# C-bowman/inference-tools

Measured on AMD Instinct MI355X. Metric: GpRegressor fit+predict wall-time and GFLOP/s at N=16384, d=8; % fp64 MFMA peak, higher is better.
Workload: dtype f64

## Files before the change

inference-tools_amd/csrc/api.hip:

```cpp
#include "api_internal.h"
#include <malloc.h>


thread_local std::string g_create_err;


int lane_streams(gpmi_ctx* c, Lane& L) {
  const size_t index = c->lanes.size() - 1;
  L.owns_stream = index < 2;
  if (!L.owns_stream) L.stream = c->lanes[index % 2].stream;
  if (L.owns_stream) HIPCHK(c, hipStreamCreateWithFlags(&L.stream, hipStreamNonBlocking));
  hipDeviceProp_t prop;
  HIPCHK(c, hipGetDeviceProperties(&prop, c->device));
  c->ncu = prop.multiProcessorCount;
  HIPCHK(c, hipEventCreateWithFlags(&L.ev_la, hipEventDisableTiming));
  HIPCHK(c, hipEventCreateWithFlags(&L.ev_panel, hipEventDisableTiming));
  HIPCHK(c, hipEventCreateWithFlags(&L.ev_join, hipEventDisableTiming));
  HIPCHK(c, hipEventCreateWithFlags(&L.ev_main, hipEventDisableTiming));
  HIPCHK(c, hipEventCreateWithFlags(&L.ev_slice, hipEventDisableTiming));
  return GPMI_OK;
}


bool ensure_masked_pair(gpmi_ctx* c, Lane& L, int k) {
// ... 240 lines not shown
      HIPCHK(c, hipStreamWaitEvent(su, L.ev_join, 0));
      launch_kbuild_square_part(s, p, c->x, c->n, c->np, c->noise, L.A, c->ld, 1, GPMI_OB);
      launch_kbuild_square_part(su, p, c->x, c->n, c->np, c->noise, L.A, c->ld, 2, GPMI_OB);
    } else {
      ProfScope ps(c, s, GPMI_PROF_KBUILD, 0.0, 4.0 * c->np * c->np);
      launch_kbuild_square(s, p, c->x, c->n, c->np, c->noise, L.A, c->ld, true);
    }
  }
  if (c->ycov) launch_add_full(s, L.A, c->ld, c->ycov, c->n);
  static const bool early_fill = !std::getenv("GPMI_EARLY_FILL") || std::atoi(std::getenv("GPMI_EARLY_FILL")) != 0;
  L.early = Lane::EarlyWork();
  L.early.pending = true;
  L.early.y = c->y;
  L.early.mu = mu_dev;
  L.early.mu_const = mu_const;
  L.early.r = L.vec + 2 * c->np;
  L.early.n = c->n;
  L.early.np = c->np;
  L.early.fill[0] = L.vec;
  L.early.fill[1] = backward_out;
  L.early.ident = early_identity;
  L.early.ident_ld = c->ld;
  L.identity_ready = false;
  if (!early_fill) L.early.pending = false;
  potrf_lower(c, L, L.A, c->np, c->ld, L.invD, L.info + slot, allow_lookahead);
  if (!early_fill) L.early.pending = true;
  lane_run_early(L, s);
  if (prebuild_inv2 && L.su[0] && c->np >= 4 * GPMI_OB) {
    HIPCHK(c, hipEventRecord(L.ev_join, s));
    HIPCHK(c, hipStreamWaitEvent(L.su[0], L.ev_join, 0));
    if (int rc = ensure_inv2(c, L, L.su[0])) return rc;
    HIPCHK(c, hipEventRecord(L.ev_main, L.su[0]));
  }
  trsv_forward(c, s, L.A, c->np, c->ld, L.invD, L.vec + 2 * c->np, L.vec, L.info + slot, BatchShape(), true);
  if (prebuild_inv2 && L.inv2_valid && L.su[0]) {
    HIPCHK(c, hipEventRecord(L.ev_la, s));
    HIPCHK(c, hipStreamWaitEvent(L.su[0], L.ev_la, 0));
    launch_lml_reduce(L.su[0], L.vec, L.A, c->ld, c->np, L.red + 2 * slot);
    HIPCHK(c, hipEventRecord(L.ev_main, L.su[0]));
  } else {
    launch_lml_reduce(s, L.vec, L.A, c->ld, c->np, L.red + 2 * slot);
  }
  HIPCHK(c, hipGetLastError());
  return GPMI_OK;
}

int ensure_second_matrix(gpmi_ctx* c, Lane& L) {
  if (!L.B2) HIPCHK(c, hipMalloc(&L.B2, sizeof(double) * c->np * c->ld));
  return GPMI_OK;
}

int ensure_inv2(gpmi_ctx* c, Lane& F, hipStream_t s) {
  if (F.inv2_valid) return GPMI_OK;
  const int64_t nob = (c->np / GPMI_NB + 3) / 4;
  if (!F.inv2) HIPCHK(c, hipMalloc(&F.inv2, sizeof(double) * nob * GPMI_OB * GPMI_OB));
  if (!F.inv2_t) HIPCHK(c, hipMalloc(&F.inv2_t, sizeof(double) * nob * 256 * 256));
  build_inv2(s, F.A, c->np, c->ld, F.invD, F.inv2, F.inv2_t);
// ... 598 lines not shown
```

inference-tools_amd/csrc/gemm_f64.hip:

```cpp
#include <cstdlib>

#include "gemm_tiles.h"

namespace {

using namespace gemm_tiles;

struct GemmArgs {
  double* C;
  const double* A;
  const double* B;
  int64_t ldc, lda, ldb;
  int ntr, ntc, k;
  int kskip;
  unsigned long long* stamp;
  int64_t sC, sA, sB;
  int split, tile_base;
  FlowHook hook;
  int zlocal_tiles;
  int mixed_full;
};

struct WgId {
  int wid;
  int64_t bz;
};
__device__ inline int xcd_remap(int b, int nwg);
__device__ inline WgId wg_id(int kskip, int zlocal_tiles) {
  if (zlocal_tiles > 0) {
    const int n = (int)blockIdx.x, m = n >> 3;
    return {m % zlocal_tiles, (int64_t)(m / zlocal_tiles) * 8 + (n & 7)};
  }
  return {kskip ? (int)blockIdx.x : xcd_remap(blockIdx.x, gridDim.x), (int64_t)blockIdx.z};
}


__device__ inline int xcd_remap(int b, int nwg) {
  const int q = nwg >> 3, r = nwg & 7, xcd = b & 7;
  return (xcd < r ? xcd * (q + 1) : r * (q + 1) + (xcd - r) * q) + (b >> 3);
}

template <int TILES>
__device__ inline void tile_of(int id, int ntr, int ntc, int& ti, int& tj) {
// ... 46 lines not shown
    tile_of<TILES>(g.tile_base + wid, g.ntr, g.ntc, ti, tj);
    if (TILES == TILES_RECT && (g.kskip == 2 || g.kskip == 4) && 2 * ti >= g.ntr) tj = g.ntc - 1 - tj;
  }

  const int tid = threadIdx.x;
  const bool stamp_first = g.stamp && tid == 0 && blockIdx.x < 8 && blockIdx.z == 0;
  if (stamp_first) g.stamp[blockIdx.x] = __builtin_amdgcn_s_memrealtime();
  const unsigned mid = gridDim.x >> 1;
  const bool stamp_clock = g.stamp && tid == 0 && blockIdx.x >= mid && blockIdx.x < mid + 8 && blockIdx.z == 0;
  unsigned long long c_start = 0, r_start = 0;
  if (stamp_clock) {
    r_start = __builtin_amdgcn_s_memrealtime();
    c_start = __builtin_amdgcn_s_memtime();
  }
  const int kbeg = (g.kskip == 1) ? ti * BM : (g.kskip == 4) ? tj * BN : 0;
  const int kend = (g.kskip == 2 && (tj + 1) * BN < g.k) ? (tj + 1) * BN : g.k;
  const int64_t bz = me.bz;
  const double* __restrict__ Ag = g.A + bz * g.sA + (int64_t)ti * BM * g.lda + kbeg;
  const double* __restrict__ Bg = BKN ? g.B + bz * g.sB + (int64_t)kbeg * g.ldb + (int64_t)tj * BN
                                      : g.B + bz * g.sB + (int64_t)tj * BN * g.ldb + kbeg;
  double* Cg = g.C + bz * g.sC + (int64_t)ti * BM * g.ldc + (int64_t)tj * BN;
  if constexpr (OP == OP_ASSIGN && BKN == 0 && BN == 128 && BM <= 64) {
    if (g.kskip == 3) {
      staged_tile<OP, BKN, BM, BN, CST_NT, LD_PLAIN, true>(Ag, Bg, Cg, g.lda, g.ldb, g.ldc, (kend - kbeg) / BK, smem);
    } else {
      staged_tile<OP, BKN, BM, BN>(Ag, Bg, Cg, g.lda, g.ldb, g.ldc, (kend - kbeg) / BK, smem);
    }
  } else {
    staged_tile<OP, BKN, BM, BN>(Ag, Bg, Cg, g.lda, g.ldb, g.ldc, (kend - kbeg) / BK, smem);
  }

  const bool stamp_end = g.stamp && tid == 0 && blockIdx.x + 1024 >= gridDim.x;
  if (stamp_end) {
    asm volatile("s_waitcnt vmcnt(0)" ::: "memory");
    g.stamp[8 + (__builtin_amdgcn_s_getreg(((4 - 1) << 11) | 20) & 7)] = __builtin_amdgcn_s_memrealtime();
  }
  if (stamp_clock)
    g.stamp[16 + blockIdx.x - mid] = ((__builtin_amdgcn_s_memtime() - c_start) << 32) |
                                     ((__builtin_amdgcn_s_memrealtime() - r_start) & 0xffffffffull);
}


#ifndef GPMI_DMA_WGS
#define GPMI_DMA_WGS 2
#endif
typedef __attribute__((address_space(3))) double gemm_lds_double_t;
typedef __attribute__((address_space(1))) double gemm_glb_double_t;
// ... 149 lines not shown
    } else if (!b_kmajor || op == OP_SUB) {
      bm = 64;
      bn = 64;
      if (tiles == TILES_RECT && !b_kmajor && k > 128 && big * 4 * bt.count <= m32_max && !bt.ring_order_only) bm = 32;
      static const bool bn32 = [] {
        const char* e = std::getenv("GPMI_CHAIN_BN32");
        return !e || std::atoi(e) != 0;
      }();
      if (bn32 && bm == 32 && kskip == 2 && op == OP_ASSIGN && big * 8 * bt.count <= 2 * 256) bn = 32;
    }
  }
  if (part == 0 && kskip == 4 && b_kmajor && op == OP_ASSIGN && tiles == TILES_RECT) {
    if (big * 16 * bt.count <= 2 * 256) {
      bm = 32;
      bn = 32;
    } else {
      bm = 64;
      bn = 128;
    }
  }
  if (bt.b_lower_tri && kskip == 0 && bn == 128 && bm <= 64 && ntc == 1 && k == 128 && !b_kmajor && op == OP_ASSIGN) kskip = 3;
  GemmArgs g{C, A, B, ldc, lda, ldb, ntr * (128 / bm), ntc * (128 / bn), k, kskip, stamp,
             bt.sC, bt.sA, bt.sB, part == 2 ? 1 : 0, (part == 2 || part == 3) ? (int)nfull : 0, bt.hook, 0, 0};
  int64_t nwg;
  if (tiles == TILES_RECT)
    nwg = (int64_t)g.ntr * g.ntc;
  else
    nwg = (int64_t)g.ntc * (g.ntc + 1) / 2 + (int64_t)(g.ntr - g.ntc) * g.ntc;
  if (part == 1) nwg = nfull;
  if (nend < 0 || nend > big) nend = big;
  if (part == 2) nwg = 4 * (nend - nfull);
  if (part == 3) nwg = nend - nfull;
  if (part == 4) {
    g.mixed_full = (int)nfull;
    nwg = nfull + 4 * (nend - nfull);
  }
  if (nwg <= 0) return;
  dim3 grid((unsigned)nwg, 1, (unsigned)bt.count), block(256);
  static const bool batch_xcd = [] {
    const char* e = std::getenv("GPMI_BATCH_XCD");
    return !e || std::atoi(e) != 0;
  }();
  if (batch_xcd && bt.count >= 8 && bt.count % 8 == 0 && !stamp && nwg * bt.count < (int64_t)1 << 30) {
    g.zlocal_tiles = (int)nwg;
    grid = dim3((unsigned)(nwg * bt.count), 1, 1);
  }
// ... 139 lines not shown
```

inference-tools_amd/csrc/gemm_tiles.h:

```cpp
#pragma once
#include "gpmi_internal.h"

#ifndef GPMI_C_PLAIN
#define GPMI_C_LOAD(p) __builtin_nontemporal_load(p)
#define GPMI_C_STORE(v, p) __builtin_nontemporal_store(v, p)
#else
#define GPMI_C_LOAD(p) (*(p))
#define GPMI_C_STORE(v, p) (*(p) = (v))
#endif

namespace gemm_tiles {

constexpr int CST_NT = 0, CST_SC1 = 1;
template <int CST>
__device__ __forceinline__ void c_store_begin() {
  if (CST == CST_SC1) asm volatile("s_nop 15\n\ts_nop 15" ::: "memory");
}
template <int CST>
__device__ __forceinline__ void c_store(d2_t v, d2_t* p) {
  if (CST == CST_SC1)
    asm volatile("global_store_dwordx4 %0, %1, off sc1\n\ts_nop 1" ::"v"(p), "v"(v) : "memory");
  else
    GPMI_C_STORE(v, p);
}
// ... 23 lines not shown
template <int LD>
__device__ __forceinline__ d2_t op_load2(const d2_t* p) {
  if (LD == LD_SC1) {
    const double* q = reinterpret_cast<const double*>(p);
    return d2_t{__hip_atomic_load(q, __ATOMIC_RELAXED, __HIP_MEMORY_SCOPE_AGENT),
                __hip_atomic_load(q + 1, __ATOMIC_RELAXED, __HIP_MEMORY_SCOPE_AGENT)};
  }
  return *p;
}

constexpr int BK = 16;
constexpr int LDS_STRIDE = 18;
#ifndef GPMI_SMALL_PF
#define GPMI_SMALL_PF 4
#endif

template <int BKN, int BM, int BN>
constexpr int staged_lds_doubles() {
  return 2 * (BM * LDS_STRIDE + (BKN ? BK * (BN + 16) : BN * LDS_STRIDE));
}

template <int OP, int BKN, int BM, int BN, int CST = CST_NT, int LD = LD_PLAIN, bool BTRI = false>
__device__ __forceinline__ void staged_tile(const double* __restrict__ Ag, const double* __restrict__ Bg, double* Cg,
                                            int64_t lda, int64_t ldb, int64_t ldc, int nk, double* smem) {
  static_assert(!BTRI || (BKN == 0 && BN == 128 && OP == OP_ASSIGN), "BTRI: the in-place panel TRSM only");
  constexpr int CSTEP = BTRI ? 32 : 16;
  constexpr int TM = BM / 32, TN = BN / 32;
  constexpr int LDS_STRIDE_KN = BN + 16;
  constexpr int A_DOUBLES = BM * LDS_STRIDE;
  constexpr int B_DOUBLES = BKN ? BK * LDS_STRIDE_KN : BN * LDS_STRIDE;
  constexpr int BUF_DOUBLES = A_DOUBLES + B_DOUBLES;
  const int tid = threadIdx.x;
  const int lane = tid & 63, wave = tid >> 6;
  const int wr = wave >> 1, wc = wave & 1;

  const int lrow = tid >> 3, lkc = (tid & 7) * 2;
  const int lkc_sw = lkc ^ ((((lrow & 15) >= 4) && ((lrow & 15) < 12)) ? 4 : 0);
  const int nrow = tid / (BN / 2), nnc = (tid % (BN / 2)) * 2;
  constexpr int PF = (BM * BN < 128 * 128) ? GPMI_SMALL_PF : 1;
  d2_t ra[PF][TM], rb[PF][TN];
  unsigned voa[TM], vob[TN];
#pragma unroll
  for (int i = 0; i < TM; ++i) voa[i] = (unsigned)(((int64_t)(lrow + 32 * i) * lda + lkc) * 8);
#pragma unroll
  for (int i = 0; i < TN; ++i)
    vob[i] = BKN ? (unsigned)(((int64_t)(nrow + (512 / BN) * i) * ldb + nnc) * 8)
                 : (unsigned)(((int64_t)(lrow + 32 * i) * ldb + lkc) * 8);
// ... 2 lines not shown
    const char* bb = reinterpret_cast<const char*>(BKN ? Bg + (int64_t)k0 * ldb : Bg + k0);
#pragma unroll
    for (int i = 0; i < TM; ++i) ra[slot][i] = op_load2<LD>(reinterpret_cast<const d2_t*>(ab + voa[i]));
#pragma unroll
    for (int i = 0; i < TN; ++i) rb[slot][i] = op_load2<LD>(reinterpret_cast<const d2_t*>(bb + vob[i]));
  };
  auto sstore = [&](int buf, int slot) {
    double* sa = smem + buf * BUF_DOUBLES;
    double* sb = sa + A_DOUBLES;
#pragma unroll
    for (int i = 0; i < TM; ++i)
      *reinterpret_cast<d2_t*>(sa + (lrow + 32 * i) * LDS_STRIDE + lkc_sw) = (OP == OP_SUB) ? -ra[slot][i] : ra[slot][i];
#pragma unroll
    for (int i = 0; i < TN; ++i) {
      if (BKN)
        *reinterpret_cast<d2_t*>(sb + (nrow + (512 / BN) * i) * LDS_STRIDE_KN + nnc) = rb[slot][i];
      else
        *reinterpret_cast<d2_t*>(sb + (lrow + 32 * i) * LDS_STRIDE + lkc_sw) = rb[slot][i];
    }
  };

  const int fr = lane & 15, fk = lane >> 4;
  const int wcol = BTRI ? wc * 16 : wc * (BN / 2);
  Cg += (int64_t)(wr * (BM / 2)) * ldc + wcol;
  const int sw = (fr >= 4 && fr < 12) ? 1 : 0;
  const int a_off = (wr * (BM / 2) + fr) * LDS_STRIDE + ((fk ^ sw) << 2);
  const int b_off = BKN ? 4 * fk * LDS_STRIDE_KN + wc * (BN / 2) + fr
                        : (wcol + fr) * LDS_STRIDE + ((fk ^ sw) << 2);

  const int klast = (nk - 1) * BK;
  auto gload_clamped = [&](int kt, int slot) { gload(kt < nk ? kt * BK : klast, slot); };
  if (PF == 1) gload(0, 0);
  d4_t acc[TM][TN];
#pragma unroll
  for (int i = 0; i < TM; ++i)
#pragma unroll
    for (int j = 0; j < TN; ++j) {
      if (OP == OP_SUB) {
#pragma unroll
        for (int r = 0; r < 4; ++r) acc[i][j][r] = c_load1<LD>(&Cg[(int64_t)(i * 16 + fk + 4 * r) * ldc + j * CSTEP + fr]);
      } else {
        acc[i][j] = d4_t{0.0, 0.0, 0.0, 0.0};
      }
    }
  if (PF > 1) {
    gload(0, 0);
// ... 38 lines not shown
    if (PF > 1 || kt + 1 < nk) sstore(cur ^ 1, slot_next);
    __syncthreads();
  };
  if (PF == 1) {
    kstep(0, 0, 0);
    for (int kt = 1; kt < nk; ++kt) kstep(kt, 0, 0);
  } else {
    for (int kb = 0; kb < nk; kb += PF) {
#pragma unroll
      for (int u = 0; u < PF; ++u) {
        if (kb + u >= nk) break;
        kstep(kb + u, u, (1 + u) % PF);
      }
    }
  }

  c_store_begin<CST>();
#pragma unroll
  for (int i = 0; i < TM; ++i)
#pragma unroll
    for (int j = 0; j < TN; ++j)
#pragma unroll
      for (int r = 0; r < 4; ++r) c_store<CST>(acc[i][j][r], &Cg[(int64_t)(i * 16 + fk + 4 * r) * ldc + j * CSTEP + fr]);
}

constexpr int DMA_BK = 8;
#ifndef GPMI_DMA_STAGES
#define GPMI_DMA_STAGES 4
#endif
constexpr int DMA_STAGES = GPMI_DMA_STAGES;
constexpr int DMA_OP_DOUBLES = 128 * DMA_BK;
constexpr int DMA128_LDS_DOUBLES = DMA_STAGES * 2 * DMA_OP_DOUBLES;
constexpr int DMA64_LDS_DOUBLES = DMA_STAGES * 2 * 64 * DMA_BK;

__device__ inline void dma_wait(int newer) {
  if (newer >= 12) asm volatile("s_waitcnt vmcnt(12)" ::: "memory");
  else if (newer >= 8) asm volatile("s_waitcnt vmcnt(8)" ::: "memory");
  else if (newer >= 4) asm volatile("s_waitcnt vmcnt(4)" ::: "memory");
  else asm volatile("s_waitcnt vmcnt(0)" ::: "memory");
}

template <int OP, int CST = CST_NT, int LD = LD_PLAIN>
__device__ __forceinline__ void dma128_tile(const double* __restrict__ Ag, const double* __restrict__ Bg, double* Cg,
                                            int64_t lda, int64_t ldb, int64_t ldc, int nk, double* smem) {
  const int tid = threadIdx.x, lane = tid & 63, wave = tid >> 6;
  const int wr = wave >> 1, wc = wave & 1;
// ... 336 lines not shown
```

inference-tools_amd/csrc/gpmi_internal.h:

```cpp
#pragma once
#include <hip/hip_runtime.h>
#include <cstdint>
#include <string>
#include <vector>

#include "gpmi.h"

constexpr int GPMI_NB = 128;
constexpr int GPMI_MAX_D = 64;
constexpr int GPMI_INFO_FLOW_TIMEOUT = -6;
constexpr int GPMI_NPAIRS = 1;

typedef double d2_t __attribute__((ext_vector_type(2)));
typedef double d4_t __attribute__((ext_vector_type(4)));

static inline int64_t round_up(int64_t v, int64_t m) { return (v + m - 1) / m * m; }

struct KParams {
  int kernel;
  int d;
  double a2;
  double kappa;
  double extra_diag;
  double inv_l2[GPMI_MAX_D];
// ... 180 lines not shown
void launch_scale_columns(hipStream_t s, const double* A, const double* sc, double* G, int64_t ld,
                          int64_t np, int batch = 1, int64_t sMat = 0, int64_t sVec = 0);
void launch_loo_vectors(hipStream_t s, const double* alpha, const double* ikdiag, double* c1,
                        double* sc2, int64_t n, int64_t np, int batch = 1, int64_t sAlpha = 0, int64_t sLoo = 0);

struct FlowHook {
  int* pub = nullptr;
  int pub_val = 0;
  const int* wait = nullptr;
  int wait_val = 0;
  int* abort = nullptr;
  int* info = nullptr;
  unsigned long long* wait_ticks = nullptr;
  unsigned long long* trace = nullptr;
};

struct GemmBatch {
  int count = 1;
  int64_t sC = 0, sA = 0, sB = 0;
  int ncu_hint = 0;
  bool b_lower_tri = false;
  bool ring_order_only = false;
  FlowHook hook;
};
struct BatchShape {
  int count = 1;
  int64_t sMat = 0;
  int64_t sInv = 0;
  int64_t sVec = 0;
};

constexpr int GPMI_MAX_MIX = 4;
void launch_scale_add(hipStream_t s, double* dst, int64_t ldd, const double* src, int64_t lds,
                      const double* gr, const double* gc, int64_t rows, int64_t cols, bool accumulate, int batch = 1,
                      int64_t sD = 0, int64_t sS = 0, int64_t sG = 0);
void launch_add_diag_vec(hipStream_t s, double* A, int64_t ld, const double* noise, double extra, int64_t n,
                         int batch = 1, int64_t sA = 0, const double* extras = nullptr);
void launch_vec_mul(hipStream_t s, const double* a, const double* b, double* out, int64_t n, int batch = 1,
                    int64_t sA = 0, int64_t sB = 0, int64_t sOut = 0);
void launch_mix_rowsum(hipStream_t s, const double* iK, const double* Km, int64_t ld, const double* alpha,
                       const double* g, double* h, int64_t n, int batch = 1, int64_t sMat = 0, int64_t sAlpha = 0,
                       int64_t sG = 0, const double* u = nullptr, int64_t sU = 0, int64_t pair = 0);

enum GemmTiles { TILES_RECT = 0, TILES_LOWER = 1 };
enum GemmOp { OP_SUB = 0, OP_ASSIGN = 1 };
void launch_gemm_nt(hipStream_t s, GemmTiles tiles, GemmOp op, double* C, int64_t ldc,
                    const double* A, int64_t lda, const double* B, int64_t ldb, int ntr, int ntc,
                    int k, unsigned long long* stamp = nullptr, const GemmBatch& bt = GemmBatch());

int64_t gemm_split_point(int64_t T, int ncu, int k);
bool gemm_mixed_launches();
void launch_gemm_nt_split(hipStream_t s, GemmTiles tiles, GemmOp op, double* C, int64_t ldc, const double* A,
                          int64_t lda, const double* B, int64_t ldb, int ntr, int ntc, int k, int64_t nfull,
                          unsigned long long* stamp = nullptr, unsigned long long* stamp_rest = nullptr,
                          int64_t nend = -1);
void launch_gemm_nt_range(hipStream_t s, GemmTiles tiles, GemmOp op, double* C, int64_t ldc, const double* A,
                          int64_t lda, const double* B, int64_t ldb, int ntr, int ntc, int k, int64_t first,
                          int64_t count, unsigned long long* stamp = nullptr);

void launch_gemm(hipStream_t s, GemmTiles tiles, GemmOp op, bool b_kmajor, int kskip, double* C,
                 int64_t ldc, const double* A, int64_t lda, const double* B, int64_t ldb, int ntr,
                 int ntc, int k, unsigned long long* stamp = nullptr, const GemmBatch& bt = GemmBatch());

hipStream_t potrf_first_update_stream(gpmi_ctx* c, Lane& lane, int64_t np, bool allow_lookahead);
void potrf_pair_quiesce(Lane& lane);
void launch_potrf_diag(hipStream_t s, double* Ablk, int64_t ld, double* invD, int* info, int col0,
                       unsigned long long* dbg = nullptr, const BatchShape& bs = BatchShape(), int* pub = nullptr,
                       int pub_val = 0);
void launch_potrf_diag_fault(hipStream_t s, double* Ablk, int64_t ld, const BatchShape& bs = BatchShape());
void potrf_lower_batched(gpmi_ctx* c, hipStream_t s, double* A, int64_t np, int64_t ld, double* invD,
                         int* info, const BatchShape& bs);
void launch_kbuild_square_batched(hipStream_t s, int kernel, const KParams* pdev, int batch, const double* x,
                                  int64_t n, int64_t np, const double* noise, double* A, int64_t ld,
                                  int64_t stride, int d, int64_t noise_stride = 0);
void potrf_lower(gpmi_ctx* c, Lane& lane, double* A, int64_t np, int64_t ld, double* invD,
                 int* info, bool allow_lookahead = true);

bool potrf_flow_enabled(gpmi_ctx* c, Lane& lane, int m);
bool potrf_flow_tail(gpmi_ctx* c, Lane& lane, double* A, int64_t ld, double* invD, int* info, int nt, int t0);
void potrf_flow_free(Lane& lane);

void trsv_forward(gpmi_ctx* c, hipStream_t s, const double* L, int64_t np, int64_t ld,
                  const double* invD, const double* r, double* out, int* err = nullptr,
                  const BatchShape& bs = BatchShape(), bool prefilled = false);
void trsv_backward(gpmi_ctx* c, hipStream_t s, const double* L, int64_t np, int64_t ld,
                   const double* invD, const double* r, double* out, int* err = nullptr,
                   const BatchShape& bs = BatchShape(), bool prefilled = false);
void lane_run_early(Lane& lane, hipStream_t s);
void trsm_identity_batched(hipStream_t s, const double* L, int64_t np, int64_t ld, const double* invD, double* Q,
                           const BatchShape& bs);
constexpr int GPMI_OB = 512;
void build_inv2(hipStream_t s, const double* L, int64_t np, int64_t ld, const double* invD, double* inv2,
                double* tmp);
void trsm_rows_forward(gpmi_ctx* c, hipStream_t s, const double* L, int64_t np, int64_t ld,
                       const double* inv2, double* Q, int64_t mp, bool upper_rhs, double* Qout,
                       double* panel);
void launch_set_identity(hipStream_t s, double* Q, int64_t ld, int64_t np, int batch = 1, int64_t sMat = 0);
void launch_copy(hipStream_t s, const double* src, double* dst, int64_t n);
void launch_copy_rows(hipStream_t s, const double* src, int64_t spitch, double* dst, int64_t dpitch, int64_t width,
// ... 24 lines not shown
```

inference-tools_amd/csrc/potrf.hip:

```cpp
#include <cstdlib>
#include <type_traits>
#include <utility>
#include <vector>

#include "gpmi_internal.h"
#include "potrf_diag.h"

namespace {

constexpr int NB = GPMI_NB;
using potrf_diag::DIAG_THREADS;

__global__ __launch_bounds__(DIAG_THREADS) void potrf_diag_kernel(double* __restrict__ A, int64_t ld,
                                                         double* __restrict__ invD,
                                                         int* __restrict__ info, int col0,
                                                         unsigned long long* __restrict__ dbg,
                                                         int64_t strideA, int64_t strideInv, int* pub, int pub_val) {
  if (pub && threadIdx.x == 0 && blockIdx.z == 0)
    __hip_atomic_store(pub, pub_val, __ATOMIC_RELAXED, __HIP_MEMORY_SCOPE_AGENT);
  __shared__ potrf_diag::DiagShared sh;
  potrf_diag::potrf_diag_body<false>(A + (int64_t)blockIdx.z * strideA, ld, invD + (int64_t)blockIdx.z * strideInv,
                                     info + blockIdx.z, col0, dbg, sh, potrf_diag::DiagPub());
}

}

namespace {
__global__ void fault_scale_kernel(double* A, int64_t ld, double f, int64_t strideA) {
  A += (int64_t)blockIdx.z * strideA;
  const int r = blockIdx.x, c = threadIdx.x;
  if (c <= r) A[(int64_t)r * ld + c] *= f;
}
}

void launch_potrf_diag_fault(hipStream_t s, double* Ablk, int64_t ld, const BatchShape& bs) {
  static const double fault = [] {
    const char* e = std::getenv("GPMI_FAULT_DIAG_EPS");
    return e ? std::atof(e) : 0.0;
  }();
  if (fault != 0.0)
    hipLaunchKernelGGL(fault_scale_kernel, dim3(NB, 1, (unsigned)bs.count), dim3(NB), 0, s, Ablk, ld, 1.0 + fault,
                       bs.sMat);
}

void launch_potrf_diag(hipStream_t s, double* Ablk, int64_t ld, double* invD, int* info, int col0,
                       unsigned long long* dbg, const BatchShape& bs, int* pub, int pub_val) {
  hipLaunchKernelGGL(potrf_diag_kernel, dim3(1, 1, (unsigned)bs.count), dim3(DIAG_THREADS), 0, s, Ablk, ld, invD,
                     info, col0, dbg, bs.sMat, bs.sInv, pub, pub_val);
  launch_potrf_diag_fault(s, Ablk, ld, bs);
}

namespace {

void factor_panel(gpmi_ctx* c, hipStream_t sp, double* A, int64_t ld, double* invD, int* info, int nt,
                  int J, int Je, int ncu = 0) {
  GemmBatch on;
  on.ncu_hint = ncu;
  on.b_lower_tri = true;
  static const bool trace = std::getenv("GPMI_CHAIN_TRACE") != nullptr;
  auto slot = [&](int tag) { return trace ? prof_stamp_slot(c, 0.0, 0.0, GPMI_PROF_NCLASS + tag) : nullptr; };
  for (int j = J; j < Je; ++j) {
    double* Ajj = A + (int64_t)j * NB * ld + (int64_t)j * NB;
    double* invDj = invD + (int64_t)j * NB * NB;
    const int below = nt - j - 1;
    {
      ProfScope ps(c, sp, GPMI_PROF_PANEL, (double)NB * NB * NB / 3.0 + 2.0 * below * NB * NB * NB,
                   8.0 * NB * NB * (2.0 + 2.0 * below));
      launch_potrf_diag(sp, Ajj, ld, invDj, info, j * NB, slot(0));
      if (below > 0) {
        double* A21 = Ajj + (int64_t)NB * ld;
        launch_gemm_nt(sp, TILES_RECT, OP_ASSIGN, A21, ld, A21, ld, invDj, NB, below, 1, NB, slot(1), on);
      }
    }
    const int pc = Je - j - 1;
    if (below > 0 && pc > 0) {
      double* A21 = Ajj + (int64_t)NB * ld;
      double* C = A21 + NB;
      const double tiles = pc * (pc + 1) / 2.0 + (double)(below - pc) * pc;
      ProfScope ps(c, sp, GPMI_PROF_PANEL, tiles * 2.0 * NB * NB * NB, tiles * 16.0 * NB * NB);
      launch_gemm_nt(sp, TILES_LOWER, OP_SUB, C, ld, A21, ld, A21, ld, below, pc, NB, slot(2));
    }
  }
}

void update_columns(gpmi_ctx* c, hipStream_t s, double* A, int64_t ld, int nt, int t0, int t1, int ka, int ke,
                    int ncu, int64_t slice = 0) {
  const int rows = nt - t0, cols = t1 - t0;
  const int kw = (ke - ka) * NB;
  if (rows <= 0 || cols <= 0 || kw <= 0) return;
  double* P = A + (int64_t)t0 * NB * ld + (int64_t)ka * NB;
  double* C = A + (int64_t)t0 * NB * ld + (int64_t)t0 * NB;
// ... 70 lines not shown
    const int x = e ? std::atoi(e) : 52;
    return x > 0 ? x : (1 << 30);
  }();
  return v;
}
}

void potrf_pair_quiesce(Lane& lane) {
  for (int k = 0; k < GPMI_NPAIRS; ++k)
    for (hipStream_t q : {lane.sp[k], lane.su[k]})
      if (q && hipStreamQuery(q) != hipSuccess) {
        (void)hipGetLastError();
        (void)hipStreamSynchronize(q);
      }
  lane.pair_checked = true;
}

hipStream_t potrf_first_update_stream(gpmi_ctx* c, Lane& lane, int64_t np, bool allow_lookahead) {
  const int nt = (int)(np / NB);
  if (!allow_lookahead || nt - OUTER_TILES < lookahead_min() || !ensure_masked_pair(c, lane, 0)) return nullptr;
  return lane.su[0];
}

void potrf_lower(gpmi_ctx* c, Lane& lane, double* A, int64_t np, int64_t ld, double* invD, int* info,
                 bool allow_lookahead) {
  hipStream_t sf = lane.stream;
  const int nt = (int)(np / NB);
  const int OBT = OUTER_TILES;
  const int LOOKAHEAD_MIN = lookahead_min();
  if (!lane.pair_checked) potrf_pair_quiesce(lane);
  lane.pair_checked = false;
  const bool la_ok = allow_lookahead && nt - OBT >= LOOKAHEAD_MIN && ensure_masked_pair(c, lane, 0);
  const bool flow_ok = allow_lookahead;
  if (flow_ok && !(la_ok && nt - OBT >= LOOKAHEAD_MIN) && potrf_flow_enabled(c, lane, nt) &&
      potrf_flow_tail(c, lane, A, ld, invD, info, nt, 0))
    return;
  auto follow = [](hipStream_t waiter, hipStream_t producer, hipEvent_t ev) {
    if (waiter != producer) (void)hipStreamWaitEvent(waiter, ev, 0);
  };
  auto tile0 = [&](int panel) { return panel * OBT < nt ? panel * OBT : nt; };
  const int NP = (nt + OBT - 1) / OBT;
  factor_panel(c, sf, A, ld, invD, info, nt, 0, tile0(1));
  hipStream_t panel_stream = sf;
  hipStream_t main_stream = sf;
  bool sliced = false;
  (void)hipEventRecord(lane.ev_panel, sf);
  (void)hipEventRecord(lane.ev_main, sf);
  if (la_ok && NP > 1 && nt - tile0(1) >= LOOKAHEAD_MIN) lane_run_early(lane, sf);
  for (int p = 0; p + 1 < NP; ++p) {
    const int k0 = tile0(p), k1 = tile0(p + 1);
    const int rem = nt - k1;
    const bool overlap = la_ok && rem >= LOOKAHEAD_MIN;
    hipStream_t su = overlap ? lane.su[0] : sf, sp = overlap ? lane.sp[0] : sf;
    const int ncu = overlap ? c->ncu - c->pair_cus[0] : c->ncu;
    follow(su, panel_stream, lane.ev_panel);
    follow(su, main_stream, lane.ev_main);
    int64_t slice = 0;
    if (overlap) {
      const int k2 = tile0(p + 2);
      update_columns(c, su, A, ld, nt, k1, k2, k0, k1, ncu);
      (void)hipEventRecord(lane.ev_la, su);
      (void)hipStreamWaitEvent(sp, lane.ev_la, 0);
      const int w = k2 - k1, r2 = nt - k2;
      slice = slice_tiles(rem, (int64_t)w * (w + 1) / 2 + (int64_t)(rem - w) * w, (int64_t)r2 * (r2 + 1) / 2,
                          (k1 - k0) * NB, ncu, c->pair_cus[0]);
      if (sliced) (void)hipStreamWaitEvent(su, lane.ev_slice, 0);
      update_columns(c, su, A, ld, nt, k2, nt, k0, k1, ncu, slice);
      (void)hipEventRecord(lane.ev_main, su);
    } else {
      if (sliced) (void)hipStreamWaitEvent(su, lane.ev_slice, 0);
      update_columns(c, su, A, ld, nt, k1, nt, k0, k1, ncu);
      if (flow_ok && potrf_flow_enabled(c, lane, nt - k1) && potrf_flow_tail(c, lane, A, ld, invD, info, nt, k1)) return;
    }
    sliced = false;
    main_stream = su;
    factor_panel(c, sp, A, ld, invD, info, nt, k1, tile0(p + 2), overlap ? c->pair_cus[0] : 0);
    if (overlap) (void)hipEventRecord(lane.ev_panel, sp);
    panel_stream = sp;
    if (slice > 0) {
      update_slice(c, sp, A, ld, nt, tile0(p + 2), nt, k0, k1, slice);
      (void)hipEventRecord(lane.ev_slice, sp);
      sliced = true;
    }
  }
  follow(sf, panel_stream, lane.ev_panel);
  follow(sf, main_stream, lane.ev_main);
  if (sliced) (void)hipStreamWaitEvent(sf, lane.ev_slice, 0);
}

void potrf_lower_batched(gpmi_ctx* c, hipStream_t s, double* A, int64_t np, int64_t ld, double* invD,
                         int* info, const BatchShape& bs) {
  (void)c;
  static const int OBT = [] {
    const char* e = std::getenv("GPMI_BATCH_OUTER");
    const int v = e ? std::atoi(e) : 4;
    return v > 0 ? v : 1;
  }();
  const int nt = (int)(np / NB);
  GemmBatch inplace{bs.count, bs.sMat, bs.sMat, bs.sInv};
  inplace.b_lower_tri = true;
  const GemmBatch upd{bs.count, bs.sMat, bs.sMat, bs.sMat};
  static const bool left = [] {
    const char* e = std::getenv("GPMI_BATCH_LEFT");
    return !e || std::atoi(e) != 0;
  }();
  for (int J = 0; J < nt; J += OBT) {
    const int Je = (J + OBT < nt) ? J + OBT : nt;
    for (int j = J; j < Je; ++j) {
      double* Ajj = A + (int64_t)j * NB * ld + (int64_t)j * NB;
      double* invDj = invD + (int64_t)j * NB * NB;
// ... 23 lines not shown
```

inference-tools_amd/csrc/solve.hip:

```cpp
#include <cstdlib>
#include <mutex>

#include "gpmi_internal.h"

namespace {

constexpr int NB = GPMI_NB;

__device__ inline double wave_sum(double v) {
#pragma unroll
  for (int off = 32; off > 0; off >>= 1) v += __shfl_down(v, off, 64);
  return v;
}

constexpr unsigned long long FLOW_SENTINEL = 0xFFF8DEADBEEF0000ull;
constexpr int FLOW_THREADS = 512;
constexpr int FLOW_SPIN_LIMIT = 1 << 22;

__device__ inline double flow_poll(const double* p, int* err, bool& dead) {
  const unsigned long long* q = reinterpret_cast<const unsigned long long*>(p);
  unsigned long long bits = __hip_atomic_load(q, __ATOMIC_RELAXED, __HIP_MEMORY_SCOPE_AGENT);
  int spins = 0;
  while (bits == FLOW_SENTINEL && !dead) {
    __builtin_amdgcn_s_sleep(1);
// ... 384 lines not shown
  if (workgroups <= FLOW_GATE_MIN || c->device < 0 || c->device >= 64) return;
  std::lock_guard<std::mutex> lk(g_sweep_mu);
  const int d = c->device;
  if (!g_sweep_ev[d] && hipEventCreateWithFlags(&g_sweep_ev[d], hipEventDisableTiming) != hipSuccess) {
    g_sweep_ev[d] = nullptr;
    (void)hipGetLastError();
    return;
  }
  if (g_sweep_used[d]) (void)hipStreamWaitEvent(s, g_sweep_ev[d], 0);
}
static void flow_gate_leave(gpmi_ctx* c, hipStream_t s, int64_t workgroups) {
  if (workgroups <= FLOW_GATE_MIN || c->device < 0 || c->device >= 64) return;
  std::lock_guard<std::mutex> lk(g_sweep_mu);
  const int d = c->device;
  if (!g_sweep_ev[d]) return;
  (void)hipEventRecord(g_sweep_ev[d], s);
  g_sweep_used[d] = true;
}

void lane_run_early(Lane& lane, hipStream_t s) {
  Lane::EarlyWork& e = lane.early;
  if (!e.pending) return;
  e.pending = false;
  launch_residual(s, e.y, e.mu, e.mu_const, e.r, e.n, e.np);
  for (double* f : e.fill)
    if (f) hipLaunchKernelGGL(flow_fill_kernel, dim3((unsigned)((e.np + 255) / 256), 1, 1), dim3(256), 0, s, f, e.np, (int64_t)0);
  if (e.ident) {
    launch_set_identity(s, e.ident, e.ident_ld, e.np);
    lane.identity_ready = true;
  }
}

void trsv_forward(gpmi_ctx* c, hipStream_t s, const double* L, int64_t np, int64_t ld,
                  const double* invD, const double* r, double* out, int* err, const BatchShape& bs, bool prefilled) {
  const int nt = (int)(np / NB);
  flow_gate_enter(c, s, (int64_t)nt);
  ProfScope ps(c, s, GPMI_PROF_SOLVE, (double)np * np, 4.0 * np * np);
  if (!prefilled)
    hipLaunchKernelGGL(flow_fill_kernel, dim3((unsigned)((np + 255) / 256), 1, (unsigned)bs.count), dim3(256), 0, s,
                       out, np, bs.sVec);
  const unsigned grid = bs.count > 1 ? 8u * (unsigned)nt * (unsigned)((bs.count + 7) / 8) : (unsigned)nt;
  hipLaunchKernelGGL(trsv_fwd_flow_kernel, dim3(grid), dim3(FLOW_THREADS), 0, s, L, ld, invD, r, out, err, bs.sMat,
                     bs.sInv, bs.sVec, nt, bs.count);
  flow_gate_leave(c, s, (int64_t)nt);
}

void trsv_backward(gpmi_ctx* c, hipStream_t s, const double* L, int64_t np, int64_t ld,
// ... 184 lines not shown
```

Measured before the change: 55400.

## Fuse forward substitution into the blocked Cholesky panel kernels

```diff
diff --git a/inference-tools_amd/csrc/api.hip b/inference-tools_amd/csrc/api.hip
--- a/inference-tools_amd/csrc/api.hip
+++ b/inference-tools_amd/csrc/api.hip
@@ -286,8 +286,17 @@
   L.early.ident = early_identity;
   L.early.ident_ld = c->ld;
   L.identity_ready = false;
+  static const bool fused_env = !std::getenv("GPMI_FUSED_FWD") || std::atoi(std::getenv("GPMI_FUSED_FWD")) != 0;
+  const bool fused = fused_env && potrf_first_update_stream(c, L, c->np, allow_lookahead) != nullptr;
+  double* fwd_r = L.vec + 2 * c->np;
+  if (fused) {
+    launch_residual(s, c->y, mu_dev, mu_const, fwd_r, c->n, c->np);
+    L.early.r = nullptr;
+    L.early.fill[0] = nullptr;
+  }
   if (!early_fill) L.early.pending = false;
-  potrf_lower(c, L, L.A, c->np, c->ld, L.invD, L.info + slot, allow_lookahead);
+  const int fend = potrf_lower(c, L, L.A, c->np, c->ld, L.invD, L.info + slot, allow_lookahead,
+                               fused ? fwd_r : nullptr, fused ? L.vec : nullptr);
   if (!early_fill) L.early.pending = true;
   lane_run_early(L, s);
   if (prebuild_inv2 && L.su[0] && c->np >= 4 * GPMI_OB) {
@@ -296,7 +305,12 @@
     if (int rc = ensure_inv2(c, L, L.su[0])) return rc;
     HIPCHK(c, hipEventRecord(L.ev_main, L.su[0]));
   }
-  trsv_forward(c, s, L.A, c->np, c->ld, L.invD, L.vec + 2 * c->np, L.vec, L.info + slot, BatchShape(), true);
+  {
+    const int64_t f0 = (int64_t)fend * GPMI_NB;
+    if (f0 < c->np)
+      trsv_forward(c, s, L.A + f0 * c->ld + f0, c->np - f0, c->ld, L.invD + f0 * GPMI_NB, fwd_r + f0, L.vec + f0,
+                   L.info + slot, BatchShape(), !fused);
+  }
   if (prebuild_inv2 && L.inv2_valid && L.su[0]) {
     HIPCHK(c, hipEventRecord(L.ev_la, s));
     HIPCHK(c, hipStreamWaitEvent(L.su[0], L.ev_la, 0));
diff --git a/inference-tools_amd/csrc/gemm_f64.hip b/inference-tools_amd/csrc/gemm_f64.hip
--- a/inference-tools_amd/csrc/gemm_f64.hip
+++ b/inference-tools_amd/csrc/gemm_f64.hip
@@ -1,3 +1,4 @@
+#include <cstdio>
 #include <cstdlib>
 
 #include "gemm_tiles.h"
@@ -19,6 +20,8 @@
   FlowHook hook;
   int zlocal_tiles;
   int mixed_full;
+  const double* fwd_z;
+  double* fwd_s;
 };
 
 struct WgId {
@@ -111,7 +114,8 @@
   double* Cg = g.C + bz * g.sC + (int64_t)ti * BM * g.ldc + (int64_t)tj * BN;
   if constexpr (OP == OP_ASSIGN && BKN == 0 && BN == 128 && BM <= 64) {
     if (g.kskip == 3) {
-      staged_tile<OP, BKN, BM, BN, CST_NT, LD_PLAIN, true>(Ag, Bg, Cg, g.lda, g.ldb, g.ldc, (kend - kbeg) / BK, smem);
+      staged_tile<OP, BKN, BM, BN, CST_NT, LD_PLAIN, true>(Ag, Bg, Cg, g.lda, g.ldb, g.ldc, (kend - kbeg) / BK, smem,
+                                                           g.fwd_z, g.fwd_s ? g.fwd_s + (int64_t)ti * BM : nullptr);
     } else {
       staged_tile<OP, BKN, BM, BN>(Ag, Bg, Cg, g.lda, g.ldb, g.ldc, (kend - kbeg) / BK, smem);
     }
@@ -307,6 +311,14 @@
   if (bt.b_lower_tri && kskip == 0 && bn == 128 && bm <= 64 && ntc == 1 && k == 128 && !b_kmajor && op == OP_ASSIGN) kskip = 3;
   GemmArgs g{C, A, B, ldc, lda, ldb, ntr * (128 / bm), ntc * (128 / bn), k, kskip, stamp,
              bt.sC, bt.sA, bt.sB, part == 2 ? 1 : 0, (part == 2 || part == 3) ? (int)nfull : 0, bt.hook, 0, 0};
+  if (bt.fwd_z) {
+    if (kskip != 3 || bt.count != 1 || !bt.fwd_s) {
+      std::fprintf(stderr, "gpmi: forward substitution asked of a product that is not a panel TRSM\n");
+      std::abort();
+    }
+    g.fwd_z = bt.fwd_z;
+    g.fwd_s = bt.fwd_s;
+  }
   int64_t nwg;
   if (tiles == TILES_RECT)
     nwg = (int64_t)g.ntr * g.ntc;
diff --git a/inference-tools_amd/csrc/gemm_tiles.h b/inference-tools_amd/csrc/gemm_tiles.h
--- a/inference-tools_amd/csrc/gemm_tiles.h
+++ b/inference-tools_amd/csrc/gemm_tiles.h
@@ -69,7 +69,8 @@
 
 template <int OP, int BKN, int BM, int BN, int CST = CST_NT, int LD = LD_PLAIN, bool BTRI = false>
 __device__ __forceinline__ void staged_tile(const double* __restrict__ Ag, const double* __restrict__ Bg, double* Cg,
-                                            int64_t lda, int64_t ldb, int64_t ldc, int nk, double* smem) {
+                                            int64_t lda, int64_t ldb, int64_t ldc, int nk, double* smem,
+                                            const double* __restrict__ fz = nullptr, double* fs = nullptr) {
   static_assert(!BTRI || (BKN == 0 && BN == 128 && OP == OP_ASSIGN), "BTRI: the in-place panel TRSM only");
   constexpr int CSTEP = BTRI ? 32 : 16;
   constexpr int TM = BM / 32, TN = BN / 32;
@@ -118,6 +119,14 @@
 
   const int fr = lane & 15, fk = lane >> 4;
   const int wcol = BTRI ? wc * 16 : wc * (BN / 2);
+  double zc[BTRI ? TN : 1], s_old = 0.0;
+  if constexpr (BTRI) {
+    if (fz) {
+#pragma unroll
+      for (int j = 0; j < TN; ++j) zc[j] = fz[j * CSTEP + wcol + fr];
+      if (tid < BM) s_old = fs[tid];
+    }
+  }
   Cg += (int64_t)(wr * (BM / 2)) * ldc + wcol;
   const int sw = (fr >= 4 && fr < 12) ? 1 : 0;
   const int a_off = (wr * (BM / 2) + fr) * LDS_STRIDE + ((fk ^ sw) << 2);
@@ -202,6 +211,25 @@
     for (int j = 0; j < TN; ++j)
 #pragma unroll
       for (int r = 0; r < 4; ++r) c_store<CST>(acc[i][j][r], &Cg[(int64_t)(i * 16 + fk + 4 * r) * ldc + j * CSTEP + fr]);
+  if constexpr (BTRI) {
+    if (fz) {
+#pragma clang fp contract(off)
+      double* red = smem;
+#pragma unroll
+      for (int i = 0; i < TM; ++i)
+#pragma unroll
+        for (int r = 0; r < 4; ++r) {
+          double u = acc[i][0][r] * zc[0];
+#pragma unroll
+          for (int j = 1; j < TN; ++j) u = u + acc[i][j][r] * zc[j];
+#pragma unroll
+          for (int m = 1; m < 16; m <<= 1) u = u + __shfl_xor(u, m, 16);
+          if (fr == 0) red[wc * BM + wr * (BM / 2) + i * 16 + fk + 4 * r] = u;
+        }
+      __syncthreads();
+      if (tid < BM) fs[tid] = s_old - (red[tid] + red[BM + tid]);
+    }
+  }
 }
 
 constexpr int DMA_BK = 8;
diff --git a/inference-tools_amd/csrc/gpmi_internal.h b/inference-tools_amd/csrc/gpmi_internal.h
--- a/inference-tools_amd/csrc/gpmi_internal.h
+++ b/inference-tools_amd/csrc/gpmi_internal.h
@@ -226,6 +226,8 @@
   bool b_lower_tri = false;
   bool ring_order_only = false;
   FlowHook hook;
+  const double* fwd_z = nullptr;
+  double* fwd_s = nullptr;
 };
 struct BatchShape {
   int count = 1;
@@ -270,15 +272,15 @@
 void potrf_pair_quiesce(Lane& lane);
 void launch_potrf_diag(hipStream_t s, double* Ablk, int64_t ld, double* invD, int* info, int col0,
                        unsigned long long* dbg = nullptr, const BatchShape& bs = BatchShape(), int* pub = nullptr,
-                       int pub_val = 0);
+                       int pub_val = 0, const double* fwd_s = nullptr, double* fwd_z = nullptr);
 void launch_potrf_diag_fault(hipStream_t s, double* Ablk, int64_t ld, const BatchShape& bs = BatchShape());
 void potrf_lower_batched(gpmi_ctx* c, hipStream_t s, double* A, int64_t np, int64_t ld, double* invD,
                          int* info, const BatchShape& bs);
 void launch_kbuild_square_batched(hipStream_t s, int kernel, const KParams* pdev, int batch, const double* x,
                                   int64_t n, int64_t np, const double* noise, double* A, int64_t ld,
                                   int64_t stride, int d, int64_t noise_stride = 0);
-void potrf_lower(gpmi_ctx* c, Lane& lane, double* A, int64_t np, int64_t ld, double* invD,
-                 int* info, bool allow_lookahead = true);
+int potrf_lower(gpmi_ctx* c, Lane& lane, double* A, int64_t np, int64_t ld, double* invD,
+                int* info, bool allow_lookahead = true, double* fwd_s = nullptr, double* fwd_z = nullptr);
 
 bool potrf_flow_enabled(gpmi_ctx* c, Lane& lane, int m);
 bool potrf_flow_tail(gpmi_ctx* c, Lane& lane, double* A, int64_t ld, double* invD, int* info, int nt, int t0);
diff --git a/inference-tools_amd/csrc/potrf.hip b/inference-tools_amd/csrc/potrf.hip
--- a/inference-tools_amd/csrc/potrf.hip
+++ b/inference-tools_amd/csrc/potrf.hip
@@ -1,3 +1,4 @@
+#include <algorithm>
 #include <cstdlib>
 #include <type_traits>
 #include <utility>
@@ -15,17 +16,87 @@
                                                          double* __restrict__ invD,
                                                          int* __restrict__ info, int col0,
                                                          unsigned long long* __restrict__ dbg,
-                                                         int64_t strideA, int64_t strideInv, int* pub, int pub_val) {
+                                                         int64_t strideA, int64_t strideInv, int* pub, int pub_val,
+                                                         const double* __restrict__ fs, double* __restrict__ fz) {
   if (pub && threadIdx.x == 0 && blockIdx.z == 0)
     __hip_atomic_store(pub, pub_val, __ATOMIC_RELAXED, __HIP_MEMORY_SCOPE_AGENT);
   __shared__ potrf_diag::DiagShared sh;
+  const int tid = threadIdx.x;
+  double s_pre = 0.0;
+  if (fz && tid < NB) s_pre = fs[tid];
   potrf_diag::potrf_diag_body<false>(A + (int64_t)blockIdx.z * strideA, ld, invD + (int64_t)blockIdx.z * strideInv,
                                      info + blockIdx.z, col0, dbg, sh, potrf_diag::DiagPub());
+  if (!fz) return;
+  using potrf_diag::BS;
+  using potrf_diag::WP;
+  __syncthreads();
+  double* sv = sh.S;
+  if (tid < NB) sv[tid] = s_pre;
+  __syncthreads();
+  const int r = tid >> 2, q = tid & 3, rb = r / BS;
+  double acc = 0.0;
+#pragma unroll
+  for (int h = 0; h < 2; ++h) {
+    const int jb = q + 4 * h;
+    if (jb <= rb) {
+      const double* X = sh.Xl[rb * (rb + 1) / 2 + jb] + (r % BS) * WP;
+#pragma unroll
+      for (int c = 0; c < BS; ++c) acc = __builtin_fma(X[c], sv[jb * BS + c], acc);
+    }
+  }
+  acc = acc + __shfl_xor(acc, 1, 4);
+  acc = acc + __shfl_xor(acc, 2, 4);
+  if (q == 0) fz[r] = acc;
 }
 
 }
 
 namespace {
+__global__ __launch_bounds__(DIAG_THREADS) void fwd_replay_z_kernel(const double* __restrict__ invD,
+                                                                   const double* __restrict__ fs, double* __restrict__ fz) {
+  using potrf_diag::BS;
+  const int tid = threadIdx.x;
+  const int r = tid >> 2, q = tid & 3, rb = r / BS;
+  double acc = 0.0;
+#pragma unroll
+  for (int h = 0; h < 2; ++h) {
+    const int jb = q + 4 * h;
+    if (jb <= rb) {
+      const double* X = invD + (int64_t)r * NB + jb * BS;
+#pragma unroll
+      for (int c = 0; c < BS; ++c) acc = __builtin_fma(X[c], fs[jb * BS + c], acc);
+    }
+  }
+  acc = acc + __shfl_xor(acc, 1, 4);
+  acc = acc + __shfl_xor(acc, 2, 4);
+  if (q == 0) fz[r] = acc;
+}
+
+__global__ __launch_bounds__(256) void fwd_replay_s_kernel(const double* __restrict__ Lc, int64_t ld,
+                                                          const double* __restrict__ fz, double* __restrict__ fs) {
+#pragma clang fp contract(off)
+  __shared__ double red[2 * 32];
+  const int tid = threadIdx.x, lane = tid & 63, wave = tid >> 6, wr = wave >> 1, wc = wave & 1;
+  const int fr = lane & 15, fk = lane >> 4;
+  const int64_t row0 = (int64_t)blockIdx.x * 32;
+  double zc[4];
+#pragma unroll
+  for (int j = 0; j < 4; ++j) zc[j] = fz[j * 32 + wc * 16 + fr];
+  const double s_old = tid < 32 ? fs[row0 + tid] : 0.0;
+#pragma unroll
+  for (int r = 0; r < 4; ++r) {
+    const int row = wr * 16 + fk + 4 * r;
+    const double* Lr = Lc + (row0 + row) * ld + wc * 16 + fr;
+    double u = Lr[0] * zc[0];
+#pragma unroll
+    for (int j = 1; j < 4; ++j) u = u + Lr[j * 32] * zc[j];
+#pragma unroll
+    for (int m = 1; m < 16; m <<= 1) u = u + __shfl_xor(u, m, 16);
+    if (fr == 0) red[wc * 32 + row] = u;
+  }
+  __syncthreads();
+  if (tid < 32) fs[row0 + tid] = s_old - (red[tid] + red[32 + tid]);
+}
 __global__ void fault_scale_kernel(double* A, int64_t ld, double f, int64_t strideA) {
   A += (int64_t)blockIdx.z * strideA;
   const int r = blockIdx.x, c = threadIdx.x;
@@ -44,16 +115,18 @@
 }
 
 void launch_potrf_diag(hipStream_t s, double* Ablk, int64_t ld, double* invD, int* info, int col0,
-                       unsigned long long* dbg, const BatchShape& bs, int* pub, int pub_val) {
+                       unsigned long long* dbg, const BatchShape& bs, int* pub, int pub_val, const double* fwd_s,
+                       double* fwd_z) {
+  if (bs.count != 1) fwd_z = nullptr;
   hipLaunchKernelGGL(potrf_diag_kernel, dim3(1, 1, (unsigned)bs.count), dim3(DIAG_THREADS), 0, s, Ablk, ld, invD,
-                     info, col0, dbg, bs.sMat, bs.sInv, pub, pub_val);
+                     info, col0, dbg, bs.sMat, bs.sInv, pub, pub_val, fwd_s, fwd_z);
   launch_potrf_diag_fault(s, Ablk, ld, bs);
 }
 
 namespace {
 
 void factor_panel(gpmi_ctx* c, hipStream_t sp, double* A, int64_t ld, double* invD, int* info, int nt,
-                  int J, int Je, int ncu = 0) {
+                  int J, int Je, int ncu = 0, double* fs = nullptr, double* fz = nullptr, int fend = 0) {
   GemmBatch on;
   on.ncu_hint = ncu;
   on.b_lower_tri = true;
@@ -66,7 +139,11 @@
     {
       ProfScope ps(c, sp, GPMI_PROF_PANEL, (double)NB * NB * NB / 3.0 + 2.0 * below * NB * NB * NB,
                    8.0 * NB * NB * (2.0 + 2.0 * below));
-      launch_potrf_diag(sp, Ajj, ld, invDj, info, j * NB, slot(0));
+      const bool fwd = fz && j < fend;
+      launch_potrf_diag(sp, Ajj, ld, invDj, info, j * NB, slot(0), BatchShape(), nullptr, 0,
+                        fwd ? fs + (int64_t)j * NB : nullptr, fwd ? fz + (int64_t)j * NB : nullptr);
+      on.fwd_z = fwd ? fz + (int64_t)j * NB : nullptr;
+      on.fwd_s = fwd ? fs + (int64_t)(j + 1) * NB : nullptr;
       if (below > 0) {
         double* A21 = Ajj + (int64_t)NB * ld;
         launch_gemm_nt(sp, TILES_RECT, OP_ASSIGN, A21, ld, A21, ld, invDj, NB, below, 1, NB, slot(1), on);
@@ -183,8 +260,8 @@
   return lane.su[0];
 }
 
-void potrf_lower(gpmi_ctx* c, Lane& lane, double* A, int64_t np, int64_t ld, double* invD, int* info,
-                 bool allow_lookahead) {
+int potrf_lower(gpmi_ctx* c, Lane& lane, double* A, int64_t np, int64_t ld, double* invD, int* info,
+                bool allow_lookahead, double* fwd_s, double* fwd_z) {
   hipStream_t sf = lane.stream;
   const int nt = (int)(np / NB);
   const int OBT = OUTER_TILES;
@@ -193,15 +270,40 @@
   lane.pair_checked = false;
   const bool la_ok = allow_lookahead && nt - OBT >= LOOKAHEAD_MIN && ensure_masked_pair(c, lane, 0);
   const bool flow_ok = allow_lookahead;
+  constexpr int FOLD_ROWS = 52;
+  int fend = 0, head_end = 0;
+  if (fwd_s && fwd_z && la_ok) {
+    fend = head_end = nt;
+    for (int k1 = OBT; k1 < nt; k1 += OBT)
+      if (nt - k1 < FOLD_ROWS) {
+        fend = k1;
+        break;
+      }
+    for (int k1 = OBT; k1 < nt; k1 += OBT)
+      if (nt - k1 < LOOKAHEAD_MIN) {
+        head_end = k1;
+        break;
+      }
+  }
+  auto replay = [&]() {
+    for (int j = head_end; j < fend; ++j) {
+      hipLaunchKernelGGL(fwd_replay_z_kernel, dim3(1), dim3(DIAG_THREADS), 0, sf, invD + (int64_t)j * NB * NB,
+                         fwd_s + (int64_t)j * NB, fwd_z + (int64_t)j * NB);
+      if (j + 1 < nt)
+        hipLaunchKernelGGL(fwd_replay_s_kernel, dim3((unsigned)((nt - j - 1) * (NB / 32))), dim3(256), 0, sf,
+                           A + (int64_t)(j + 1) * NB * ld + (int64_t)j * NB, ld, fwd_z + (int64_t)j * NB,
+                           fwd_s + (int64_t)(j + 1) * NB);
+    }
+  };
   if (flow_ok && !(la_ok && nt - OBT >= LOOKAHEAD_MIN) && potrf_flow_enabled(c, lane, nt) &&
       potrf_flow_tail(c, lane, A, ld, invD, info, nt, 0))
-    return;
+    return fend;
   auto follow = [](hipStream_t waiter, hipStream_t producer, hipEvent_t ev) {
     if (waiter != producer) (void)hipStreamWaitEvent(waiter, ev, 0);
   };
   auto tile0 = [&](int panel) { return panel * OBT < nt ? panel * OBT : nt; };
   const int NP = (nt + OBT - 1) / OBT;
-  factor_panel(c, sf, A, ld, invD, info, nt, 0, tile0(1));
+  factor_panel(c, sf, A, ld, invD, info, nt, 0, tile0(1), 0, fwd_s, fwd_z, std::min(fend, head_end));
   hipStream_t panel_stream = sf;
   hipStream_t main_stream = sf;
   bool sliced = false;
@@ -231,11 +333,15 @@
     } else {
       if (sliced) (void)hipStreamWaitEvent(su, lane.ev_slice, 0);
       update_columns(c, su, A, ld, nt, k1, nt, k0, k1, ncu);
-      if (flow_ok && potrf_flow_enabled(c, lane, nt - k1) && potrf_flow_tail(c, lane, A, ld, invD, info, nt, k1)) return;
+      if (flow_ok && potrf_flow_enabled(c, lane, nt - k1) && potrf_flow_tail(c, lane, A, ld, invD, info, nt, k1)) {
+        replay();
+        return fend;
+      }
     }
     sliced = false;
     main_stream = su;
-    factor_panel(c, sp, A, ld, invD, info, nt, k1, tile0(p + 2), overlap ? c->pair_cus[0] : 0);
+    factor_panel(c, sp, A, ld, invD, info, nt, k1, tile0(p + 2), overlap ? c->pair_cus[0] : 0, fwd_s, fwd_z,
+                 std::min(fend, head_end));
     if (overlap) (void)hipEventRecord(lane.ev_panel, sp);
     panel_stream = sp;
     if (slice > 0) {
@@ -247,6 +353,8 @@
   follow(sf, panel_stream, lane.ev_panel);
   follow(sf, main_stream, lane.ev_main);
   if (sliced) (void)hipStreamWaitEvent(sf, lane.ev_slice, 0);
+  replay();
+  return fend;
 }
 
 void potrf_lower_batched(gpmi_ctx* c, hipStream_t s, double* A, int64_t np, int64_t ld, double* invD,
diff --git a/inference-tools_amd/csrc/solve.hip b/inference-tools_amd/csrc/solve.hip
--- a/inference-tools_amd/csrc/solve.hip
+++ b/inference-tools_amd/csrc/solve.hip
@@ -430,7 +430,7 @@
   Lane::EarlyWork& e = lane.early;
   if (!e.pending) return;
   e.pending = false;
-  launch_residual(s, e.y, e.mu, e.mu_const, e.r, e.n, e.np);
+  if (e.r) launch_residual(s, e.y, e.mu, e.mu_const, e.r, e.n, e.np);
   for (double* f : e.fill)
     if (f) hipLaunchKernelGGL(flow_fill_kernel, dim3((unsigned)((e.np + 255) / 256), 1, 1), dim3(256), 0, s, f, e.np, (int64_t)0);
   if (e.ident) {
```

New measurement: 55720, median of 6. No clear change (+0.6%).
